# HarrisonKramer/optiland

Hardware: NVIDIA H100
Metric: ray-surface intersections/sec (higher is better)
Workload: dtype f32

## Files before the change

__graft_entry__.py:

```python
from __future__ import annotations

import os
import subprocess
import sys

ROOT = os.path.dirname(os.path.abspath(__file__))
if ROOT not in sys.path:
    sys.path.insert(0, ROOT)

CSRC = os.path.join(ROOT, "optiland_b200", "csrc")
LIB = os.path.join(ROOT, "optiland_b200", "libolb.so")
NVCC_FLAGS = [
    "-gencode", "arch=compute_90a,code=sm_90a", "-lineinfo", "-O3", "-std=c++17",
    "--shared", "-Xcompiler", "-fPIC",
]


def _stale(target: str, deps: list[str]) -> bool:
    if not os.path.exists(target):
        return True
    t = os.path.getmtime(target)
    return any(os.path.getmtime(d) > t for d in deps)


def build(force: bool = False) -> None:
    deps = [os.path.join(CSRC, f) for f in ("olb_trace.cu", "olb_math.cuh", "olb_prep.h", "olb_psf.cu", "olb_fftpsf.cuh",
                                            "olb_irradiance.cu", "olb_irradiance.cuh", "olb_bsdf.cuh", "olb_aim.cuh")]
    deps.append(os.path.join(ROOT, "include", "olb.h"))
    if force or _stale(LIB, deps):
        nvcc = os.environ.get("NVCC", "/usr/local/cuda/bin/nvcc")
        cmd = [nvcc, *NVCC_FLAGS, "-o", LIB, os.path.join(CSRC, "olb_trace.cu"), os.path.join(CSRC, "olb_psf.cu"),
               os.path.join(CSRC, "olb_irradiance.cu")]
        print("[build]", " ".join(cmd), flush=True)
        subprocess.check_call(cmd)
    hc_src = os.path.join(ROOT, "tests", "hostcheck", "hostcheck.cpp")
    hc_so = os.path.join(ROOT, "tests", "hostcheck", "_hostcheck.so")
    if force or _stale(hc_so, [hc_src] + deps[1:3] + [deps[4]]):
        subprocess.check_call(["g++", "-O2", "-std=c++17", "-mfma", "-ffp-contract=fast", "-shared", "-fPIC", "-o", hc_so, hc_src])
    from oracle import hostcheck_phase

    hostcheck_phase.build(force)
    from oracle import hostcheck_grating

    hostcheck_grating.build(force)
    from oracle import hostcheck_coating

    hostcheck_coating.build(force)
    from oracle import hostcheck_grid_sag

    hostcheck_grid_sag.build(force)
    from oracle import hostcheck_polygon

    hostcheck_polygon.build(force)
    from oracle import hostcheck_bsdf

    hostcheck_bsdf.build(force)
    from oracle import hostcheck_aim

    hostcheck_aim.build(force)
    from oracle import hostcheck_irradiance

    hostcheck_irradiance.build(force)
    subprocess.check_call(["bash", os.path.join(ROOT, "oracle", "make_ref.sh")])
    import optiland_b200
    from optiland_b200 import _lib

    _lib.load()


def smoke() -> None:
    import numpy as np
    import torch

    from oracle import trace_oracle as O
    from optiland_b200.trace import RealRays, SurfaceGroup
    from tests._util import REC, Case, max_abs_err

    assert torch.cuda.is_available(), "smoke() needs a CUDA device"
    c = Case("dgauss_c2")
    _, orec, _ = O.trace(c.table, c.rays)
    for dtype, tol in ((torch.float64, 1e-11 * c.scale), (torch.float32, 2e-6 * c.scale)):
        sg = SurfaceGroup(c.table, device="cuda:0")
        r = c.rays
        rays = RealRays(r["x"], r["y"], r["z"], r["L"], r["M"], r["N"], r["i"], r["w"], dtype=dtype, device="cuda:0")
        sg.trace(rays)
        torch.cuda.synchronize()
        for k in REC:
            got = getattr(sg, k).double().cpu().numpy()
            err_o = max_abs_err(got, orec[k])
            err_g = max_abs_err(got, c.rec[k])
            assert err_o <= tol and err_g <= tol, (str(dtype), k, err_o, err_g, tol)
        print(f"[smoke] {dtype}: 13 surfaces x {c.n} rays match oracle + golden within {tol:.2e} mm")
    from oracle.ref_import import reference_available

    if reference_available():
        from oracle.ref_import import import_reference

        import_reference()
        import optiland.backend as be
        from optiland.samples.objectives import DoubleGauss

        from optiland_b200 import _lib, plugin

        be.set_backend("numpy")
        ref = DoubleGauss()
        ref.trace(Hx=0.0, Hy=0.7, wavelength=0.5876, num_rays=8, distribution="hexapolar")
        want = np.array(ref.surfaces.y)
        be.set_backend("torch")
        be.set_device("cuda")
        be.set_precision("float64")
        be.grad_mode.disable()
        plugin.install()
        try:
            l0 = _lib.load().olb_launch_count()
            lens = DoubleGauss()
            lens.trace(Hx=0.0, Hy=0.7, wavelength=0.5876, num_rays=8, distribution="hexapolar")
            got = be.to_numpy(lens.surfaces.y)
            assert _lib.load().olb_launch_count() > l0 and not plugin.stats(), plugin.stats()
            assert np.max(np.abs(got - want)) <= 1e-11 * c.scale
            print("[smoke] unmodified Optic.trace through the plugin == NumPy reference (one fused launch)")
        finally:
            plugin.uninstall()
            be.set_device("cpu")
            be.set_backend("numpy")
    print("[smoke] ok")


if __name__ == "__main__":
    build()
    if len(sys.argv) > 1 and sys.argv[1] == "smoke":
        smoke()
```

include/olb.h:

```cpp
#ifndef OLB_H_
#define OLB_H_

#include <stdint.h>

#ifdef __cplusplus
extern "C" {
#endif

#define OLB_VERSION_MAJOR 0
#define OLB_VERSION_MINOR 3

#define OLB_OK                 0
#define OLB_ERR_INVALID_ARG   -1
#define OLB_ERR_UNSUPPORTED   -2
#define OLB_ERR_CUDA          -3
#define OLB_ERR_ALIGNMENT     -4
#define OLB_ERR_TABLE         -5

#define OLB_GEOM_NOOP          0
#define OLB_GEOM_PLANE         1
#define OLB_GEOM_STANDARD      2
#define OLB_GEOM_EVEN_ASPHERE  3
#define OLB_GEOM_ZERNIKE       4
#define OLB_GEOM_ODD_ASPHERE   5
#define OLB_GEOM_POLYNOMIAL    6
#define OLB_GEOM_CHEBYSHEV     7
#define OLB_GEOM_BICONIC       8
#define OLB_GEOM_TOROIDAL      9
#define OLB_GEOM_FORBES_QBFS  10
#define OLB_GEOM_GRID_SAG     11
#define OLB_MAX_GRID_ELEMENTS 8192


#define OLB_SF_REFLECT     (1u << 0)
#define OLB_SF_ROTATED     (1u << 1)
#define OLB_SF_APERTURE    (1u << 2)
#define OLB_SF_ABSORBING   (1u << 3)
#define OLB_SF_NORECORD    (1u << 4)
#define OLB_SF_BSDF        (1u << 5)

#define OLB_BSDF_LAMBERTIAN 1
#define OLB_BSDF_GAUSSIAN   2
#define OLB_BSDF_MAX_ATTEMPTS 65536

#define OLB_COAT_NONE      0
#define OLB_COAT_SIMPLE    1
#define OLB_COAT_FRESNEL   2
#define OLB_COAT_THIN_FILM 3
#define OLB_COAT_POLARIZER 4
#define OLB_COAT_RETARDER  5
#define OLB_MAX_FILM_LAYERS 32

#define OLB_INTERACT_REFRACT        0
#define OLB_INTERACT_PHASE_CONSTANT 1
#define OLB_INTERACT_PHASE_LINEAR   2
#define OLB_INTERACT_PHASE_RADIAL   3
#define OLB_INTERACT_GRATING        4
#define OLB_MAX_PHASE_TERMS        16

#define OLB_AP_RADIAL      1
#define OLB_AP_OFFSET_RADIAL 2
#define OLB_AP_RECT        3
#define OLB_AP_ELLIPSE     4
#define OLB_AP_POLYGON     5
#define OLB_AP_UNION       16
#define OLB_AP_INTERSECT   17
#define OLB_AP_DIFFERENCE  18
#define OLB_MAX_POLYGON_VERTICES 1024

#define OLB_TF_POLARIZED   (1u << 0)
#define OLB_TF_POL_IDENTITY (1u << 2)
#define OLB_TF_SHARED_INPUT (1u << 4)
#define OLB_TF_MOMENTS     (1u << 3)
#define OLB_TF_MOMENTS_GLOBAL (1u << 5)
#define OLB_TF_MOMENTS_ALL (1u << 6)
#define OLB_TF_NO_FINAL    (1u << 1)

#define OLB_MAX_SURFACES   64
#define OLB_MAX_WAVELENGTHS 16

typedef struct OlbSurface {
  int32_t kind;
  uint32_t flags;
  int32_t n_coef;
  int32_t coef_off;
  int32_t aper_off;
  int32_t aper_len;
  int32_t max_iter;
  int32_t coating;
  int32_t media_off;
  int32_t aux0;
  int32_t interaction;
  int32_t phase_off;
  double t[3];
  double R[9];
  double radius;
  double conic;
  double tol;
  double coat_t;
  double coat_r;
  double norm_radius;
} OlbSurface;


typedef struct OlbTable {
  const OlbSurface* surfaces;
  int32_t n_surfaces;
  int32_t n_wl;
  const double* wavelengths;
  const double* pool;
  int32_t pool_len;
  int32_t reserved;
} OlbTable;

typedef struct OlbRays {
  void* x; void* y; void* z;
  void* L; void* M; void* N;
  void* i; void* w; void* opd;
  void* L0; void* M0; void* N0;
  void* p;
} OlbRays;

typedef struct OlbRecords {
  void* x; void* y; void* z;
  void* L; void* M; void* N;
  void* intensity; void* opd;
  int64_t row_stride;
} OlbRecords;

#define OLB_ST_CHEBYSHEV_RANGE (1 << 1)
#define OLB_ST_ZERNIKE_RANGE (1 << 0)

#define OLB_ST_K_PARALLEL_X (1 << 2)
#define OLB_ST_BSDF_ATTEMPTS (1 << 3)
#define OLB_ST_AIM_NAN_START (1 << 4)
#define OLB_ST_AIM_UNCONVERGED (1 << 5)

int olb_version(void);
int olb_last_error(char* buf, int buf_len);

typedef struct OlbDeviceTable {
  void* workspace;
  int64_t workspace_bytes;
  uint32_t magic;
  uint32_t features;
  int32_t n_surfaces;
  int32_t n_wl;
  int32_t off_f64, bytes_f64;
  int32_t off_f32, bytes_f32;
  int32_t bwd_supported;
  int32_t bwd_slots;
  int32_t n_systems;
  int32_t stride_f64;
  int32_t stride_f32;
  int32_t hints;
} OlbDeviceTable;

int64_t olb_table_workspace_bytes(const OlbTable* table);

int olb_table_upload(const OlbTable* table, void* workspace, int64_t workspace_bytes,
                     void* stream, OlbDeviceTable* out);

typedef struct OlbPupilLaunch {
  const void* Px;
  const void* Py;
  double origin0[3];
  double origin_scale[2];
  double target0[3];
  double target_scale[2];
  double intensity;
  const void* Hx;
  const void* Hy;
  int32_t field_mode;
  int32_t n_vig;
  double field_arg;
  double origin_field[2];
  double target_field[2];
  int32_t vig_power;
  int32_t reserved;
  double vig[16][4];
} OlbPupilLaunch;
#define OLB_MAX_VIG_FIELDS 16

int64_t olb_host_scratch_bytes(int32_t elem_size, int64_t chunk_rays);
int olb_trace_host_f32(const OlbDeviceTable* table, int32_t first, int32_t last,
                       const OlbPupilLaunch* launch, const OlbRays* h_in, const OlbRays* h_out,
                       const OlbRecords* rec, int64_t n_rays, int64_t chunk_rays,
                       void* dev_scratch, int64_t dev_scratch_bytes, uint32_t flags,
                       int32_t* status);
int olb_trace_host_f64(const OlbDeviceTable* table, int32_t first, int32_t last,
                       const OlbPupilLaunch* launch, const OlbRays* h_in, const OlbRays* h_out,
                       const OlbRecords* rec, int64_t n_rays, int64_t chunk_rays,
                       void* dev_scratch, int64_t dev_scratch_bytes, uint32_t flags,
                       int32_t* status);

#define OLB_GP_TX 0
#define OLB_GP_TY 1
#define OLB_GP_TZ 2
#define OLB_GP_CURV 3
#define OLB_GP_CONIC 4
#define OLB_GP_N1 5
#define OLB_GP_N2 6
#define OLB_GP_COEF 7
#define OLB_GP_MAX_COEF 12
#define OLB_GP_R (OLB_GP_COEF + OLB_GP_MAX_COEF)
#define OLB_GP_COUNT (OLB_GP_R + 9)

#define OLB_GT_DIM 12
#define OLB_GT_PER_SURFACE (2 * OLB_GT_DIM * OLB_GT_DIM)
int olb_trace_bwd_f32(const OlbDeviceTable* table, int32_t first, int32_t last,
                      const OlbRays* rays_in, const OlbRecords* rec, const OlbRecords* grad_rec,
                      const OlbRays* grad_rays_in, double* grad_params, double* grad_tables, int64_t n_rays,
                      uint64_t grad_row_mask, void* stream);
int olb_trace_bwd_f64(const OlbDeviceTable* table, int32_t first, int32_t last,
                      const OlbRays* rays_in, const OlbRecords* rec, const OlbRecords* grad_rec,
                      const OlbRays* grad_rays_in, double* grad_params, double* grad_tables, int64_t n_rays,
                      uint64_t grad_row_mask, void* stream);

typedef struct {
  double center[3];
  double radius;
  double n_image;
  double tilt[2];
  double opd_ref;
  double wavelength_um;
} OlbWavefrontRef;
typedef struct {
  void* opd;
  void* pupil_x;
  void* pupil_y;
  void* pupil_z;
  void* intensity;
} OlbWavefrontOut;

typedef struct OlbPolarization {
  int32_t is_polarized;
  int32_t reserved;
  double Ex, Ey;
  double phase_x, phase_y;
  void* intensity;
} OlbPolarization;

#define OLB_BP_TX 0
#define OLB_BP_TY 1
#define OLB_BP_TZ 2
#define OLB_BP_R 3
#define OLB_BP_CURV 12
#define OLB_BP_CONIC 13
#define OLB_BP_N1 14
#define OLB_BP_N2 15
#define OLB_BP_COEF 16
#define OLB_BP_MAX_COEF 12
#define OLB_BP_COUNT (OLB_BP_COEF + OLB_BP_MAX_COEF)
int64_t olb_table_batch_workspace_bytes(const OlbTable* template_table, int32_t n_systems);
int olb_table_upload_batch(const OlbTable* template_table, const double* params, int32_t n_systems,
                           void* workspace, int64_t workspace_bytes, void* stream, OlbDeviceTable* out);

typedef struct OlbTraceCall {
  int32_t first, last;
  int64_t n_rays;
  uint32_t flags;
  uint32_t rng_stream;
  const OlbRays* rays;
  const OlbRecords* rec;
  const OlbPupilLaunch* launch;
  double center[2];
  double* moments;
  int64_t rays_per_system;
  const OlbWavefrontRef* wavefront_ref;
  const OlbWavefrontOut* wavefront_out;
  const OlbPolarization* pol;
  int32_t* status;
} OlbTraceCall;
int olb_trace_call_f32(const OlbDeviceTable* table, const OlbTraceCall* call, void* stream);
int olb_trace_call_f64(const OlbDeviceTable* table, const OlbTraceCall* call, void* stream);

typedef struct OlbAimCall {
  int32_t first, last;
  int64_t n_rays;
  const OlbRays* rays;
  const void* Px;
  const void* Py;
  double r_stop;
  double J_factor;
  double tol;
  int32_t max_iter;
  int32_t infinite;
  int32_t* status;
} OlbAimCall;
int olb_aim_f32(const OlbDeviceTable* table, const OlbAimCall* call, void* stream);
int olb_aim_f64(const OlbDeviceTable* table, const OlbAimCall* call, void* stream);

int olb_huygens_psf_f64(const double* image_x, const double* image_y, const double* image_z, int64_t n_image,
                        const double* pupil_x, const double* pupil_y, const double* pupil_z,
                        const double* pupil_amp_re, const double* pupil_amp_im, const double* pupil_opd,
                        int32_t n_pupil, double wavelength_mm, double Rp, double* psf, double* field,
                        void* stream);

int olb_fft_pupil_f64(const double* opd_waves, const double* intensity, int64_t n_samples, const int32_t* cell_ray,
                      int32_t num_rays, int32_t grid_size, double* pupil, void* stream);
int olb_fft_pupil_f32(const float* opd_waves, const float* intensity, int64_t n_samples, const int32_t* cell_ray,
                      int32_t num_rays, int32_t grid_size, float* pupil, void* stream);
int olb_fft_psf_accumulate_f64(const double* amp, int32_t grid_size, int32_t first, int32_t last, double div, double mul,
                               double* psf, void* stream);
int olb_fft_psf_accumulate_f32(const float* amp, int32_t grid_size, int32_t first, int32_t last, double div, double mul,
                               float* psf, void* stream);

#define OLB_IRR_FRAME_TRANSLATE 0
#define OLB_IRR_FRAME_AFFINE    1
#define OLB_IRR_PATH_AUTO   0
#define OLB_IRR_PATH_SHARED 1
#define OLB_IRR_PATH_GLOBAL 2
typedef struct OlbIrradiance {
  const void* x;
  const void* y;
  const void* z;
  const void* i;
  int64_t n_rays;
  int32_t frame;
  int32_t nx, ny;
  int32_t path;
  double t[3];
  double R[9];
  const double* x_edges;
  const double* y_edges;
  double* edges;
  double* hist;
} OlbIrradiance;
int olb_irradiance_f32(const OlbIrradiance* call, void* stream);
int olb_irradiance_f64(const OlbIrradiance* call, void* stream);

int64_t olb_launch_count(void);

#ifdef __cplusplus
}
#endif
#endif
```

optiland_b200/_lib.py:

```python
from __future__ import annotations

import ctypes as C
import os
from functools import lru_cache

import numpy as np

from . import table as T

_HERE = os.path.dirname(os.path.abspath(__file__))
LIB_PATH = os.path.join(_HERE, "libolb.so")

OK = 0
ERRORS = {-1: "OLB_ERR_INVALID_ARG", -2: "OLB_ERR_UNSUPPORTED", -3: "OLB_ERR_CUDA",
          -4: "OLB_ERR_ALIGNMENT", -5: "OLB_ERR_TABLE"}

TF_POLARIZED = 1 << 0
TF_NO_FINAL = 1 << 1
TF_POL_IDENTITY = 1 << 2
TF_MOMENTS = 1 << 3
TF_SHARED_INPUT = 1 << 4
TF_MOMENTS_GLOBAL = 1 << 5
TF_MOMENTS_ALL = 1 << 6
BP_TX, BP_TY, BP_TZ, BP_R, BP_CURV, BP_CONIC, BP_N1, BP_N2, BP_COEF, BP_MAX_COEF = 0, 1, 2, 3, 12, 13, 14, 15, 16, 12
BP_COUNT = BP_COEF + BP_MAX_COEF
GP_TX, GP_TY, GP_TZ, GP_CURV, GP_CONIC, GP_N1, GP_N2, GP_COEF, GP_MAX_COEF = 0, 1, 2, 3, 4, 5, 6, 7, 12
GP_R = GP_COEF + GP_MAX_COEF
GP_COUNT = GP_R + 9
GT_DIM = 12
GT_PER_SURFACE = 2 * GT_DIM * GT_DIM


class OlbTable(C.Structure):
    _fields_ = [
        ("surfaces", C.c_void_p), ("n_surfaces", C.c_int32), ("n_wl", C.c_int32),
        ("wavelengths", C.c_void_p), ("pool", C.c_void_p), ("pool_len", C.c_int32),
        ("reserved", C.c_int32),
    ]


class OlbRays(C.Structure):
    _fields_ = [(n, C.c_void_p) for n in
                ("x", "y", "z", "L", "M", "N", "i", "w", "opd", "L0", "M0", "N0", "p")]


class OlbRecords(C.Structure):
    _fields_ = [(n, C.c_void_p) for n in ("x", "y", "z", "L", "M", "N", "intensity", "opd")] + [
        ("row_stride", C.c_int64)]


class OlbPupilLaunch(C.Structure):
    _fields_ = [("Px", C.c_void_p), ("Py", C.c_void_p), ("origin0", C.c_double * 3), ("origin_scale", C.c_double * 2),
                ("target0", C.c_double * 3), ("target_scale", C.c_double * 2), ("intensity", C.c_double),
                ("Hx", C.c_void_p), ("Hy", C.c_void_p), ("field_mode", C.c_int32), ("n_vig", C.c_int32),
                ("field_arg", C.c_double), ("origin_field", C.c_double * 2), ("target_field", C.c_double * 2),
                ("vig_power", C.c_int32), ("reserved", C.c_int32), ("vig", (C.c_double * 4) * 16)]


class OlbWavefrontRef(C.Structure):
    _fields_ = [("center", C.c_double * 3), ("radius", C.c_double), ("n_image", C.c_double), ("tilt", C.c_double * 2),
                ("opd_ref", C.c_double), ("wavelength_um", C.c_double)]


class OlbWavefrontOut(C.Structure):
    _fields_ = [(n, C.c_void_p) for n in ("opd", "pupil_x", "pupil_y", "pupil_z", "intensity")]


class OlbPolarization(C.Structure):
    _fields_ = [("is_polarized", C.c_int32), ("reserved", C.c_int32), ("Ex", C.c_double), ("Ey", C.c_double),
                ("phase_x", C.c_double), ("phase_y", C.c_double), ("intensity", C.c_void_p)]


class OlbTraceCall(C.Structure):
    _fields_ = [("first", C.c_int32), ("last", C.c_int32), ("n_rays", C.c_int64), ("flags", C.c_uint32),
                ("rng_stream", C.c_uint32), ("rays", C.POINTER(OlbRays)), ("rec", C.POINTER(OlbRecords)),
                ("launch", C.POINTER(OlbPupilLaunch)), ("center", C.c_double * 2), ("moments", C.c_void_p),
                ("rays_per_system", C.c_int64), ("wavefront_ref", C.POINTER(OlbWavefrontRef)),
                ("wavefront_out", C.POINTER(OlbWavefrontOut)), ("pol", C.POINTER(OlbPolarization)),
                ("status", C.c_void_p)]


class OlbAimCall(C.Structure):
    _fields_ = [("first", C.c_int32), ("last", C.c_int32), ("n_rays", C.c_int64), ("rays", C.POINTER(OlbRays)),
                ("Px", C.c_void_p), ("Py", C.c_void_p), ("r_stop", C.c_double), ("J_factor", C.c_double),
                ("tol", C.c_double), ("max_iter", C.c_int32), ("infinite", C.c_int32), ("status", C.c_void_p)]


class OlbIrradiance(C.Structure):
    _fields_ = [("x", C.c_void_p), ("y", C.c_void_p), ("z", C.c_void_p), ("i", C.c_void_p), ("n_rays", C.c_int64),
                ("frame", C.c_int32), ("nx", C.c_int32), ("ny", C.c_int32), ("path", C.c_int32),
                ("t", C.c_double * 3), ("R", C.c_double * 9), ("x_edges", C.c_void_p), ("y_edges", C.c_void_p),
                ("edges", C.c_void_p), ("hist", C.c_void_p)]


IRR_FRAME_TRANSLATE, IRR_FRAME_AFFINE = 0, 1
IRR_PATH_AUTO, IRR_PATH_SHARED, IRR_PATH_GLOBAL = 0, 1, 2


class OlbDeviceTable(C.Structure):
    _fields_ = [
        ("workspace", C.c_void_p), ("workspace_bytes", C.c_int64), ("magic", C.c_uint32),
        ("features", C.c_uint32), ("n_surfaces", C.c_int32), ("n_wl", C.c_int32),
        ("off_f64", C.c_int32), ("bytes_f64", C.c_int32), ("off_f32", C.c_int32),
        ("bytes_f32", C.c_int32), ("bwd_supported", C.c_int32), ("bwd_slots", C.c_int32),
        ("n_systems", C.c_int32), ("stride_f64", C.c_int32), ("stride_f32", C.c_int32), ("hints", C.c_int32),
    ]


_P = C.POINTER
SYMBOLS = {
    "olb_version": (C.c_int, []),
    "olb_last_error": (C.c_int, [C.c_char_p, C.c_int]),
    "olb_launch_count": (C.c_int64, []),
    "olb_table_workspace_bytes": (C.c_int64, [_P(OlbTable)]),
    "olb_table_upload": (C.c_int, [_P(OlbTable), C.c_void_p, C.c_int64, C.c_void_p, _P(OlbDeviceTable)]),
    "olb_trace_call_f32": (C.c_int, [_P(OlbDeviceTable), _P(OlbTraceCall), C.c_void_p]),
    "olb_trace_call_f64": (C.c_int, [_P(OlbDeviceTable), _P(OlbTraceCall), C.c_void_p]),
    "olb_aim_f32": (C.c_int, [_P(OlbDeviceTable), _P(OlbAimCall), C.c_void_p]),
    "olb_aim_f64": (C.c_int, [_P(OlbDeviceTable), _P(OlbAimCall), C.c_void_p]),
    "olb_trace_bwd_f32": (C.c_int, [_P(OlbDeviceTable), C.c_int32, C.c_int32, _P(OlbRays), _P(OlbRecords),
                                    _P(OlbRecords), _P(OlbRays), C.c_void_p, C.c_void_p, C.c_int64, C.c_uint64,
                                    C.c_void_p]),
    "olb_trace_bwd_f64": (C.c_int, [_P(OlbDeviceTable), C.c_int32, C.c_int32, _P(OlbRays), _P(OlbRecords),
                                    _P(OlbRecords), _P(OlbRays), C.c_void_p, C.c_void_p, C.c_int64, C.c_uint64,
                                    C.c_void_p]),
    "olb_table_batch_workspace_bytes": (C.c_int64, [_P(OlbTable), C.c_int32]),
    "olb_table_upload_batch": (C.c_int, [_P(OlbTable), C.c_void_p, C.c_int32, C.c_void_p, C.c_int64, C.c_void_p,
                                         _P(OlbDeviceTable)]),
    "olb_huygens_psf_f64": (C.c_int, [C.c_void_p, C.c_void_p, C.c_void_p, C.c_int64, C.c_void_p, C.c_void_p, C.c_void_p,
                                      C.c_void_p, C.c_void_p, C.c_void_p, C.c_int32, C.c_double, C.c_double,
                                      C.c_void_p, C.c_void_p, C.c_void_p]),
    "olb_fft_pupil_f64": (C.c_int, [C.c_void_p, C.c_void_p, C.c_int64, C.c_void_p, C.c_int32, C.c_int32, C.c_void_p, C.c_void_p]),
    "olb_fft_pupil_f32": (C.c_int, [C.c_void_p, C.c_void_p, C.c_int64, C.c_void_p, C.c_int32, C.c_int32, C.c_void_p, C.c_void_p]),
    "olb_fft_psf_accumulate_f64": (C.c_int, [C.c_void_p, C.c_int32, C.c_int32, C.c_int32, C.c_double, C.c_double, C.c_void_p, C.c_void_p]),
    "olb_fft_psf_accumulate_f32": (C.c_int, [C.c_void_p, C.c_int32, C.c_int32, C.c_int32, C.c_double, C.c_double, C.c_void_p, C.c_void_p]),
    "olb_irradiance_f32": (C.c_int, [_P(OlbIrradiance), C.c_void_p]),
    "olb_irradiance_f64": (C.c_int, [_P(OlbIrradiance), C.c_void_p]),
    "olb_host_scratch_bytes": (C.c_int64, [C.c_int32, C.c_int64]),
    "olb_trace_host_f32": (C.c_int, [_P(OlbDeviceTable), C.c_int32, C.c_int32, _P(OlbPupilLaunch), _P(OlbRays),
                                     _P(OlbRays), _P(OlbRecords), C.c_int64, C.c_int64, C.c_void_p, C.c_int64,
                                     C.c_uint32, C.c_void_p]),
    "olb_trace_host_f64": (C.c_int, [_P(OlbDeviceTable), C.c_int32, C.c_int32, _P(OlbPupilLaunch), _P(OlbRays),
                                     _P(OlbRays), _P(OlbRecords), C.c_int64, C.c_int64, C.c_void_p, C.c_int64,
                                     C.c_uint32, C.c_void_p]),
}


class OlbError(RuntimeError):
    pass


@lru_cache(maxsize=1)
def load() -> C.CDLL:
    if not os.path.exists(LIB_PATH):
        raise OlbError(
            f"{LIB_PATH} not found: build it with `python -c 'import __graft_entry__ as g; g.build()'` "
            "(nvcc, sm_90a).  optiland_b200 has no CPU fallback.")
    lib = C.CDLL(LIB_PATH)
    for name, (restype, argtypes) in SYMBOLS.items():
        fn = getattr(lib, name)
        fn.restype = restype
        fn.argtypes = argtypes
    return lib


def last_error() -> str:
    buf = C.create_string_buffer(512)
    load().olb_last_error(buf, len(buf))
    return buf.value.decode("utf-8", "replace")


def check(rc: int, what: str) -> None:
    if rc != OK:
        raise OlbError(f"{what} failed: {ERRORS.get(rc, rc)}: {last_error()}")


class HostTable:

    def __init__(self, tab: T.SurfaceTable, packed=None):
        self.surf, self.pool = packed if packed is not None else tab.pack()
        self.surf = np.ascontiguousarray(self.surf)
        self.pool = np.ascontiguousarray(self.pool)
        self.wl = np.ascontiguousarray(tab.wavelengths, dtype=np.float64)
        self.c = OlbTable(
            surfaces=self.surf.ctypes.data, n_surfaces=len(self.surf), n_wl=len(self.wl),
            wavelengths=self.wl.ctypes.data, pool=self.pool.ctypes.data, pool_len=len(self.pool),
            reserved=0)
```

optiland_b200/trace.py:

```python
from __future__ import annotations

import ctypes as C
import threading

import numpy as np
import torch

from . import _lib
from . import table as T

_REC_KEYS = ("x", "y", "z", "L", "M", "N", "intensity", "opd")
_DTYPES = {torch.float32: "f32", torch.float64: "f64"}
_CDTYPES = {torch.float32: torch.complex64, torch.float64: torch.complex128}


def _require_cuda():
    if not torch.cuda.is_available():
        raise _lib.OlbError("optiland_b200 needs a CUDA device (sm_90a); there is no CPU fallback")


def _as_dev(v, n, dtype, device):
    t = torch.as_tensor(v, dtype=dtype, device=device)
    if t.ndim == 0:
        t = t.expand(n)
    t = t.reshape(-1).contiguous()
    if t.data_ptr() % 16:
        t = t.clone()
    return t


class RealRays:

    def __init__(self, x, y, z, L, M, N, intensity, wavelength, dtype=torch.float32, device=None):
        _require_cuda()
        if dtype not in _DTYPES:
            raise ValueError("dtype must be torch.float32 or torch.float64")
        device = torch.device(device if device is not None else f"cuda:{torch.cuda.current_device()}")
        n = max(int(np.size(v)) if not torch.is_tensor(v) else v.numel()
                for v in (x, y, z, L, M, N, intensity, wavelength))
        self.x = _as_dev(x, n, dtype, device)
        self.y = _as_dev(y, n, dtype, device)
        self.z = _as_dev(z, n, dtype, device)
        self.L = _as_dev(L, n, dtype, device)
        self.M = _as_dev(M, n, dtype, device)
        self.N = _as_dev(N, n, dtype, device)
        self.i = _as_dev(intensity, n, dtype, device)
        self.w = _as_dev(wavelength, n, dtype, device)
        self.opd = torch.zeros_like(self.x)
        self.L0 = self.M0 = self.N0 = None
        self.is_normalized = True

    def __len__(self):
        return self.x.numel()

    @property
    def dtype(self):
        return self.x.dtype

    @property
    def device(self):
        return self.x.device


class PolarizedRays(RealRays):

    def __init__(self, x, y, z, L, M, N, intensity, wavelength, dtype=torch.float32, device=None):
        super().__init__(x, y, z, L, M, N, intensity, wavelength, dtype=dtype, device=device)
        self.p = None
        self._i0 = self.i.clone()
        self._L0, self._M0, self._N0 = self.L.clone(), self.M.clone(), self.N.clone()

    def update_intensity(self, state=None):
        k = torch.stack([self._L0, self._M0, self._N0], dim=1)
        xh = torch.tensor([1.0, 0.0, 0.0], dtype=k.dtype, device=k.device).expand_as(k)
        pv = torch.linalg.cross(k, xh)
        norms = torch.linalg.norm(pv, dim=1)
        if bool((norms == 0).any()):
            raise ValueError("k-vector parallel to x-axis is not currently supported.")
        pv = pv / norms[:, None]
        sv = torch.linalg.cross(pv, k)
        states = [state] if state is not None else [(1.0, 0.0, 0.0, 0.0), (0.0, 1.0, 0.0, 0.0)]
        inten = torch.zeros_like(self._i0)
        P = self.p
        for Ex, Ey, phx, phy in states:
            ax = complex(np.cos(phx), np.sin(phx)) * Ex
            ay = complex(np.cos(phy), np.sin(phy)) * Ey
            E0 = sv.to(P.dtype) * ax + pv.to(P.dtype) * ay
            E1 = torch.matmul(P, E0[:, :, None])[:, :, 0]
            inten = inten + (E1.abs() ** 2).sum(dim=1)
        self.i = inten * self._i0 / len(states)


class DeviceTable:

    DEFAULT_WORKSPACE = 48 * 1024

    def __init__(self, table: T.SurfaceTable, device=None, packed=None):
        _require_cuda()
        self.lib = _lib.load()
        self.table = table
        self.device = torch.device(device if device is not None else f"cuda:{torch.cuda.current_device()}")
        self.host = _lib.HostTable(table, packed)
        self.c = _lib.OlbDeviceTable()
        nbytes = self.DEFAULT_WORKSPACE
        for attempt in range(2):
            self.workspace = torch.empty(int(nbytes), dtype=torch.uint8, device=self.device)
            with torch.cuda.device(self.device):
                stream = torch.cuda.current_stream(self.device).cuda_stream
                rc = self.lib.olb_table_upload(C.byref(self.host.c), self.workspace.data_ptr(), int(nbytes),
                                               C.c_void_p(stream), C.byref(self.c))
            if rc != 0 and attempt == 0 and "workspace too small" in _lib.last_error():
                nbytes = self.lib.olb_table_workspace_bytes(C.byref(self.host.c))
                if nbytes < 0:
                    _lib.check(int(nbytes), "olb_table_workspace_bytes")
                continue
            break
        _lib.check(rc, "olb_table_upload")
        self.ready = torch.cuda.Event()
        self.ready.record(torch.cuda.current_stream(self.device))
        self.has_zernike = any(s.kind in (T.GEOM_ZERNIKE, T.GEOM_CHEBYSHEV) for s in table.surfaces)
        self.has_bsdf = any(s.bsdf != T.BSDF_NONE for s in table.surfaces)

    @property
    def features(self) -> int:
        return int(self.c.features)


def _byref(s):
    return C.byref(s) if s is not None else None


def _pointer(s):
    return C.pointer(s) if s is not None else None


def _status_word(dtab: "DeviceTable", device, force: bool = False):
    return torch.zeros(1, dtype=torch.int32, device=device) if (dtab.has_zernike or _has_bsdf(dtab) or force) else None


def _has_bsdf(dtab) -> bool:
    return getattr(dtab, "has_bsdf", False)


_STREAM = {"state": None, "next": 0}
_STREAM_LOCK = threading.Lock()


def next_rng_stream() -> int:
    g = torch.default_generator
    with _STREAM_LOCK:
        st = g.get_state()
        if _STREAM["state"] is None or not torch.equal(st, _STREAM["state"]):
            _STREAM["next"] = int(torch.randint(0, 1 << 32, (1,), dtype=torch.int64).item())
            _STREAM["state"] = g.get_state()
        s = _STREAM["next"]
        _STREAM["next"] = (s + 1) & 0xFFFFFFFF
        return s


def _raise_status(status) -> None:
    if status is None:
        return
    st = int(status.item())
    if st & T.ST_ZERNIKE_RANGE:
        raise ValueError(
            "Zernike coordinates must be normalized to [-1, 1]. Consider updating the normalization "
            "radius to 1.1x the surface aperture.")
    if st & T.ST_CHEBYSHEV_RANGE:
        raise ValueError(
            "Chebyshev input coordinates must be normalized to [-1, 1]. Consider updating the "
            "normalization factors.")
    if st & T.ST_K_PARALLEL_X:
        raise ValueError("k-vector parallel to x-axis is not currently supported.")
    if st & T.ST_BSDF_ATTEMPTS:
        raise ValueError(f"BSDF scatter: a ray rejected {T.BSDF_MAX_ATTEMPTS} drawn directions (is the Gaussian sigma "
                         "far above 1?); its direction is NaN")


def _out_buffer(k: int, rows: int, n: int, dtype, device) -> torch.Tensor:
    vec = 4 if dtype == torch.float32 else 2
    stride = n if n % vec == 0 else (n + 63) // 64 * 64
    return torch.empty((k, rows, stride), dtype=dtype, device=device)


def _c_records(buf: torch.Tensor):
    return _lib.OlbRecords(*[buf[j].data_ptr() for j in range(8)], buf.shape[-1])


def _take_last_row(rays, recs):
    rays.x, rays.y, rays.z = recs["x"][-1], recs["y"][-1], recs["z"][-1]
    rays.L, rays.M, rays.N = recs["L"][-1], recs["M"][-1], recs["N"][-1]
    rays.i, rays.opd = recs["intensity"][-1], recs["opd"][-1]
    return rays


def _trace(dtab, device, dtype, first, last, n, flags, rays=None, rec=None, launch=None, center=(0.0, 0.0),
           moments=None, rays_per_system=0, wavefront=None, pol=None, status=None, own_status=True, rng_stream=None):
    if _has_bsdf(dtab) and rng_stream is None:
        rng_stream = next_rng_stream()
    if own_status:
        status = _status_word(dtab, device, force=pol is not None)
    ref, out = wavefront if wavefront is not None else (None, None)
    call = _lib.OlbTraceCall(
        first=first, last=last, n_rays=n, flags=flags, rng_stream=int(rng_stream or 0), rays=_pointer(rays),
        rec=_pointer(rec), launch=_pointer(launch),
        center=(float(center[0]), float(center[1])), moments=moments.data_ptr() if moments is not None else None,
        rays_per_system=rays_per_system, wavefront_ref=_pointer(ref), wavefront_out=_pointer(out), pol=_pointer(pol),
        status=status.data_ptr() if status is not None else None)
    sfx = _DTYPES[dtype]
    with torch.cuda.device(device):
        stream = torch.cuda.current_stream(device).cuda_stream
        rc = getattr(dtab.lib, f"olb_trace_call_{sfx}")(C.byref(dtab.c), C.byref(call), C.c_void_p(stream))
    _lib.check(rc, f"olb_trace_call_{sfx}")
    if own_status:
        _raise_status(status)


def _c_polarization(state, intensity_out=None):
    c = _lib.OlbPolarization()
    if state is None or state == "unpolarized":
        c.is_polarized = 0
    else:
        Ex, Ey, phx, phy = (float(v) for v in state)
        mag = (Ex * Ex + Ey * Ey) ** 0.5
        c.is_polarized, c.Ex, c.Ey, c.phase_x, c.phase_y = 1, Ex / mag, Ey / mag, phx, phy
    c.intensity = intensity_out.data_ptr() if intensity_out is not None else None
    return c


def trace_device(dtab: DeviceTable, rays: RealRays, first: int, last: int, record: bool = True,
                 want_l0: bool = False, polarization=False, rng_stream=None):
    n = len(rays)
    if rays.device != dtab.device:
        raise ValueError(f"rays on {rays.device}, table on {dtab.device}")
    rows = last - first
    recs = None
    c_rec = None
    flags = 0
    if record and rows > 0:
        buf = _out_buffer(8, rows, n, rays.dtype, rays.device)
        recs = {k: buf[j, :, :n] for j, k in enumerate(_REC_KEYS)}
        c_rec = _c_records(buf)
        flags |= _lib.TF_NO_FINAL
    if want_l0:
        rays.L0 = torch.empty_like(rays.x)
        rays.M0 = torch.empty_like(rays.x)
        rays.N0 = torch.empty_like(rays.x)
    p_ptr = None
    if isinstance(rays, PolarizedRays):
        flags |= _lib.TF_POLARIZED
        if rays.p is None:
            rays.p = torch.empty((n, 3, 3), dtype=_CDTYPES[rays.dtype], device=rays.device)
            flags |= _lib.TF_POL_IDENTITY
        else:
            rays.p = rays.p.to(_CDTYPES[rays.dtype]).contiguous()
        p_ptr = torch.view_as_real(rays.p).data_ptr()
    c_rays = _lib.OlbRays(
        x=rays.x.data_ptr(), y=rays.y.data_ptr(), z=rays.z.data_ptr(), L=rays.L.data_ptr(),
        M=rays.M.data_ptr(), N=rays.N.data_ptr(), i=rays.i.data_ptr(),
        w=rays.w.data_ptr() if dtab.table.n_wl > 1 else None, opd=rays.opd.data_ptr(),
        L0=rays.L0.data_ptr() if want_l0 else None, M0=rays.M0.data_ptr() if want_l0 else None,
        N0=rays.N0.data_ptr() if want_l0 else None, p=p_ptr)
    pol_i, c_pol = None, None
    if polarization is not False:
        if not isinstance(rays, PolarizedRays):
            raise ValueError("the intensity epilogue needs PolarizedRays")
        pol_i = torch.empty_like(rays.x)
        c_pol = _c_polarization(polarization, pol_i)
    _trace(dtab, rays.device, rays.dtype, first, last, n, flags, rays=c_rays, rec=c_rec, pol=c_pol, rng_stream=rng_stream)
    if recs is not None:
        _take_last_row(rays, recs)
    if pol_i is not None:
        rays.i = pol_i
    return recs


def aim_device(dtab: DeviceTable, guess: dict, Px: torch.Tensor, Py: torch.Tensor, first: int, last: int,
               r_stop: float, J_factor: float, tol: float, max_iter: int, infinite: bool) -> torch.Tensor:
    x = guess["x"]
    n = int(x.numel())
    for t in [guess[k] for k in ("y", "z", "L", "M", "N")] + [Px, Py]:
        if t.dtype != x.dtype or t.device != dtab.device or t.numel() != n:
            raise ValueError("aim: guess and pupil arrays must share one dtype, length and the table's device")
    status = torch.zeros(1, dtype=torch.int32, device=dtab.device)
    w = guess.get("w") if dtab.table.n_wl > 1 else None
    c_rays = _lib.OlbRays(x=x.data_ptr(), y=guess["y"].data_ptr(), z=guess["z"].data_ptr(), L=guess["L"].data_ptr(),
                          M=guess["M"].data_ptr(), N=guess["N"].data_ptr(), w=w.data_ptr() if w is not None else None)
    call = _lib.OlbAimCall(first=first, last=last, n_rays=n, rays=C.pointer(c_rays), Px=Px.data_ptr(), Py=Py.data_ptr(),
                           r_stop=float(r_stop), J_factor=float(J_factor), tol=float(tol), max_iter=int(max_iter),
                           infinite=1 if infinite else 0, status=status.data_ptr())
    sfx = _DTYPES[x.dtype]
    with torch.cuda.device(dtab.device):
        stream = torch.cuda.current_stream(dtab.device).cuda_stream
        rc = getattr(dtab.lib, f"olb_aim_{sfx}")(C.byref(dtab.c), C.byref(call), C.c_void_p(stream))
    _lib.check(rc, f"olb_aim_{sfx}")
    return status


def _aligned(t):
    if t is None:
        return None
    t = t.contiguous()
    return t.clone() if t.data_ptr() % 16 else t


def _c_launch(affine: dict, Px, Py):
    la = _lib.OlbPupilLaunch()
    la.Px, la.Py = Px.data_ptr(), Py.data_ptr()
    la.origin0 = (C.c_double * 3)(*affine["origin0"])
    la.origin_scale = (C.c_double * 2)(*affine["origin_scale"])
    la.target0 = (C.c_double * 3)(*affine["target0"])
    la.target_scale = (C.c_double * 2)(*affine["target_scale"])
    la.intensity = float(affine.get("intensity", 1.0))
    fields = affine.get("fields")
    if fields is not None:
        Hx, Hy = fields
        la.Hx, la.Hy = Hx.data_ptr(), Hy.data_ptr()
        la.field_mode = int(affine["field_mode"])
        la.field_arg = float(affine.get("field_arg", 0.0))
        la.origin_field = (C.c_double * 2)(*affine["origin_field"])
        la.target_field = (C.c_double * 2)(*affine["target_field"])
        vig = affine.get("vig")
        if vig is not None:
            tab, power = vig
            tab = np.asarray(tab, dtype=np.float64).reshape(-1, 4)
            if len(tab) > 16:
                raise ValueError("more than 16 defined fields with vignetting factors")
            la.n_vig, la.vig_power = len(tab), int(power)
            for j, row in enumerate(tab):
                for q in range(4):
                    la.vig[j][q] = float(row[q])
    return la


def trace_pupil_device(dtab: DeviceTable, Px: torch.Tensor, Py: torch.Tensor, affine: dict, first: int, last: int,
                       wavelength: torch.Tensor | None = None, polarization=False):
    Px, Py, wavelength = _aligned(Px), _aligned(Py), _aligned(wavelength)
    if affine.get("fields") is not None:
        affine = dict(affine, fields=tuple(_aligned(t) for t in affine["fields"]))
    n, dtype, dev = Px.numel(), Px.dtype, Px.device
    buf = _out_buffer(8, last - first, n, dtype, dev)
    recs = {k: buf[j, :, :n] for j, k in enumerate(_REC_KEYS)}
    la = _c_launch(affine, Px.contiguous(), Py.contiguous())
    out = _lib.OlbRays(w=wavelength.data_ptr() if (wavelength is not None and dtab.table.n_wl > 1) else None)
    flags = _lib.TF_NO_FINAL
    p, inten, c_pol = None, None, None
    if polarization is not False:
        flags |= _lib.TF_POLARIZED
        p = torch.empty((n, 3, 3), dtype=_CDTYPES[dtype], device=dev)
        out.p = torch.view_as_real(p).data_ptr()
        if polarization != "matrix":
            inten = torch.empty(n, dtype=dtype, device=dev)
            c_pol = _c_polarization(polarization, inten)
    _trace(dtab, dev, dtype, first, last, n, flags, rays=out, rec=_c_records(buf), launch=la, pol=c_pol)
    cls = RealRays if p is None else PolarizedRays
    rays = _take_last_row(cls.__new__(cls), recs)
    if p is not None:
        rays.p = p
    if inten is not None:
        rays.i = inten
    rays.w = wavelength
    rays.L0 = rays.M0 = rays.N0 = None
    rays.is_normalized = True
    return rays, recs


WAVEFRONT_KEYS = ("opd", "pupil_x", "pupil_y", "pupil_z", "intensity")


def trace_wavefront_device(dtab: DeviceTable, Px: torch.Tensor, Py: torch.Tensor, affine: dict, ref: dict,
                           wavelength: torch.Tensor | None = None, polarized: bool = False) -> dict:
    Px, Py, wavelength = _aligned(Px), _aligned(Py), _aligned(wavelength)
    n, dtype, dev = Px.numel(), Px.dtype, Px.device
    buf = _out_buffer(5, 1, n, dtype, dev)[:, 0]
    c_out = _lib.OlbWavefrontOut(*[buf[j].data_ptr() for j in range(5)])
    c_ref = _lib.OlbWavefrontRef()
    c_ref.center = (C.c_double * 3)(*[float(v) for v in ref["center"]])
    c_ref.radius, c_ref.n_image = float(ref["radius"]), float(ref["n_image"])
    c_ref.tilt = (C.c_double * 2)(*[float(v) for v in ref.get("tilt", (0.0, 0.0))])
    c_ref.opd_ref, c_ref.wavelength_um = float(ref["opd_ref"]), float(ref["wavelength_um"])
    la = _c_launch(affine, Px.contiguous(), Py.contiguous())
    rays = _lib.OlbRays(w=wavelength.data_ptr() if (wavelength is not None and dtab.table.n_wl > 1) else None)
    flags = _lib.TF_NO_FINAL
    p = None
    if polarized:
        flags |= _lib.TF_POLARIZED
        p = torch.empty((n, 3, 3), dtype=_CDTYPES[dtype], device=dev)
        rays.p = torch.view_as_real(p).data_ptr()
    _trace(dtab, dev, dtype, 0, dtab.table.num_surfaces, n, flags, rays=rays, launch=la, wavefront=(c_ref, c_out))
    out = {k: buf[j, :n] for j, k in enumerate(WAVEFRONT_KEYS)}
    if p is not None:
        out["p"] = p
    return out


def trace_moments_device(dtab: DeviceTable, n: int, dtype, rays: RealRays | None = None, pupil=None,
                         center=(0.0, 0.0), moments: torch.Tensor | None = None, wavelength=None,
                         status: torch.Tensor | None = None, last: int | None = None, global_xy: bool = False,
                         every_ray: bool = False) -> torch.Tensor:
    dev = dtab.device
    if moments is None:
        moments = torch.zeros(8, dtype=torch.float64, device=dev)
    la = None
    c_rays = _lib.OlbRays()
    if pupil is not None:
        Px, Py, affine = pupil
        Px, Py, wavelength = _aligned(Px), _aligned(Py), _aligned(wavelength)
        la = _c_launch(affine, Px, Py)
        if wavelength is not None and dtab.table.n_wl > 1:
            c_rays.w = wavelength.data_ptr()
    else:
        for k in ("x", "y", "z", "L", "M", "N", "i", "opd"):
            setattr(c_rays, k, getattr(rays, k).data_ptr())
        if dtab.table.n_wl > 1:
            c_rays.w = rays.w.data_ptr()
    flags = _lib.TF_NO_FINAL | (_lib.TF_MOMENTS_GLOBAL if global_xy else 0) | (_lib.TF_MOMENTS_ALL if every_ray else 0)
    _trace(dtab, dev, dtype, 0, dtab.table.num_surfaces if last is None else last, n, flags, rays=c_rays, launch=la,
           center=center, moments=moments, status=status, own_status=status is None)
    return moments


def moments_to_spot(m, center=(0.0, 0.0)) -> dict:
    m = [float(v) for v in (m.cpu() if torch.is_tensor(m) else m)]
    cnt = m[0]
    if cnt == 0:
        return {"count": 0.0}
    mx, my = m[1] / cnt, m[2] / cnt
    var_c = max(m[3] / cnt - mx * mx - my * my, 0.0)
    opd_mean = m[5] / cnt
    return {"count": cnt, "centroid": (center[0] + mx, center[1] + my), "rms_centroid": var_c ** 0.5,
            "rms_center": (m[3] / cnt) ** 0.5, "intensity_sum": m[4], "opd_mean": opd_mean,
            "opd_rms": max(m[6] / cnt - opd_mean * opd_mean, 0.0) ** 0.5}


class SurfaceGroup:

    def __init__(self, table: T.SurfaceTable, device=None):
        self.table = table
        self.device_table = DeviceTable(table, device)
        self._rec = None

    @property
    def num_surfaces(self) -> int:
        return self.table.num_surfaces

    def trace(self, rays: RealRays, skip: int = 0, stop: int | None = None, record: bool = True):
        last = self.num_surfaces if stop is None else stop
        if not 0 <= skip <= last <= self.num_surfaces:
            raise ValueError("bad surface range")
        self._rec = trace_device(self.device_table, rays, skip, last, record=record)
        return rays

    def trace_pupil(self, Px, Py, affine: dict, wavelength=None):
        rays, self._rec = trace_pupil_device(self.device_table, Px, Py, affine, 0, self.num_surfaces, wavelength)
        return rays

    def spot_moments(self, rays=None, pupil=None, center=(0.0, 0.0), dtype=None):
        if pupil is not None:
            n, dt = pupil[0].numel(), pupil[0].dtype
        else:
            n, dt = len(rays), rays.dtype
        m = trace_moments_device(self.device_table, n, dtype or dt, rays=rays, pupil=pupil, center=center)
        out = moments_to_spot(m, center)
        cen = out.get("centroid")
        if cen is not None and np.isfinite(cen[0]) and np.isfinite(cen[1]):
            m2 = trace_moments_device(self.device_table, n, dtype or dt, rays=rays, pupil=pupil, center=cen)
            out["rms_centroid"] = moments_to_spot(m2, cen)["rms_centroid"]
        return out

    def _get(self, key):
        if self._rec is None:
            raise RuntimeError("no records: call trace(..., record=True) first")
        return self._rec[key]

    x = property(lambda self: self._get("x"))
    y = property(lambda self: self._get("y"))
    z = property(lambda self: self._get("z"))
    L = property(lambda self: self._get("L"))
    M = property(lambda self: self._get("M"))
    N = property(lambda self: self._get("N"))
    opd = property(lambda self: self._get("opd"))
    intensity = property(lambda self: self._get("intensity"))


def trace_host(dtab: DeviceTable, h_in: dict, h_out: dict, n: int, dtype=torch.float32, chunk: int = 1 << 20,
               scratch: torch.Tensor | None = None, rec=None, first: int = 0, last: int | None = None,
               affine: dict | None = None):
    lib = dtab.lib
    sfx = _DTYPES[dtype]
    es = 4 if dtype == torch.float32 else 8
    last = dtab.table.num_surfaces if last is None else last
    dtab.ready.synchronize()
    need = int(lib.olb_host_scratch_bytes(es, chunk))
    if scratch is None or scratch.numel() < need:
        scratch = torch.empty(need, dtype=torch.uint8, device=dtab.device)
    c_out = _lib.OlbRays(**{k: h_out[k].data_ptr() for k in ("x", "y", "z", "L", "M", "N", "i", "opd")})
    la, c_in = None, None
    if affine is not None:
        la = _c_launch(affine, h_in["Px"], h_in["Py"])
        if dtab.table.n_wl > 1:
            c_out.w = (h_in["w"] if "w" in h_in else h_out["w"]).data_ptr()
    else:
        c_in = _lib.OlbRays(**{k: h_in[k].data_ptr() for k in ("x", "y", "z", "L", "M", "N", "i")},
                            w=h_in["w"].data_ptr() if "w" in h_in and dtab.table.n_wl > 1 else None)
    c_rec = _c_records(rec) if rec is not None else None
    status = torch.zeros(1, dtype=torch.int32, device=dtab.device) if _has_bsdf(dtab) else None
    with torch.cuda.device(dtab.device):
        rc = getattr(lib, f"olb_trace_host_{sfx}")(
            C.byref(dtab.c), first, last, _byref(la), _byref(c_in), C.byref(c_out), _byref(c_rec), n, chunk,
            C.c_void_p(scratch.data_ptr()), scratch.numel(), 0,
            C.c_void_p(status.data_ptr()) if status is not None else None)
    _lib.check(rc, f"olb_trace_host_{sfx}")
    _raise_status(status)
    return scratch
```

Baseline: 72.94 billion.

## Allocate uniform ray arrays in compressible device memory via pluggable allocator

Adds a CUDA driver-API allocator that requests generic-compression memory through cuMemCreate and exposes it to PyTorch as a MemPool. When RealRays builds its input arrays, any freshly created array whose values are all equal (for example wavelength, intensity or the zeroed OPD) is copied into this compressible memory. The aim is to cut DRAM bandwidth for these reads using hardware compression of uniform data. In exchange it adds a uniformity check with a host sync at construction, a full-device synchronize on every free, and VMM allocation overhead.

```diff
diff --git a/__graft_entry__.py b/__graft_entry__.py
--- a/__graft_entry__.py
+++ b/__graft_entry__.py
@@ -25,12 +25,13 @@
 
 def build(force: bool = False) -> None:
     deps = [os.path.join(CSRC, f) for f in ("olb_trace.cu", "olb_math.cuh", "olb_prep.h", "olb_psf.cu", "olb_fftpsf.cuh",
-                                            "olb_irradiance.cu", "olb_irradiance.cuh", "olb_bsdf.cuh", "olb_aim.cuh")]
+                                            "olb_irradiance.cu", "olb_irradiance.cuh", "olb_bsdf.cuh", "olb_aim.cuh",
+                                            "olb_alloc.cu")]
     deps.append(os.path.join(ROOT, "include", "olb.h"))
     if force or _stale(LIB, deps):
         nvcc = os.environ.get("NVCC", "/usr/local/cuda/bin/nvcc")
         cmd = [nvcc, *NVCC_FLAGS, "-o", LIB, os.path.join(CSRC, "olb_trace.cu"), os.path.join(CSRC, "olb_psf.cu"),
-               os.path.join(CSRC, "olb_irradiance.cu")]
+               os.path.join(CSRC, "olb_irradiance.cu"), os.path.join(CSRC, "olb_alloc.cu")]
         print("[build]", " ".join(cmd), flush=True)
         subprocess.check_call(cmd)
     hc_src = os.path.join(ROOT, "tests", "hostcheck", "hostcheck.cpp")
diff --git a/include/olb.h b/include/olb.h
--- a/include/olb.h
+++ b/include/olb.h
@@ -1,6 +1,7 @@
 #ifndef OLB_H_
 #define OLB_H_
 
+#include <stddef.h>
 #include <stdint.h>
 
 #ifdef __cplusplus
@@ -332,6 +333,11 @@
 
 int64_t olb_launch_count(void);
 
+int olb_compressible_supported(int device);
+void* olb_compressible_alloc(size_t size, int device, void* stream);
+void olb_compressible_free(void* ptr, size_t size, int device, void* stream);
+int olb_compressible_stats(int device, int64_t* granted_bytes, int64_t* plain_bytes);
+
 #ifdef __cplusplus
 }
 #endif
diff --git a/optiland_b200/_lib.py b/optiland_b200/_lib.py
--- a/optiland_b200/_lib.py
+++ b/optiland_b200/_lib.py
@@ -143,6 +143,10 @@
     "olb_trace_host_f64": (C.c_int, [_P(OlbDeviceTable), C.c_int32, C.c_int32, _P(OlbPupilLaunch), _P(OlbRays),
                                      _P(OlbRays), _P(OlbRecords), C.c_int64, C.c_int64, C.c_void_p, C.c_int64,
                                      C.c_uint32, C.c_void_p]),
+    "olb_compressible_supported": (C.c_int, [C.c_int]),
+    "olb_compressible_alloc": (C.c_void_p, [C.c_size_t, C.c_int, C.c_void_p]),
+    "olb_compressible_free": (None, [C.c_void_p, C.c_size_t, C.c_int, C.c_void_p]),
+    "olb_compressible_stats": (C.c_int, [C.c_int, _P(C.c_int64), _P(C.c_int64)]),
 }
 
 
diff --git a/optiland_b200/csrc/olb_alloc.cu b/optiland_b200/csrc/olb_alloc.cu
--- /dev/null
+++ b/optiland_b200/csrc/olb_alloc.cu
@@ -0,0 +1,179 @@
+#include <cuda.h>
+#include <cuda_runtime.h>
+#include <stdint.h>
+
+#include <mutex>
+#include <unordered_map>
+
+#include "../../include/olb.h"
+
+namespace olb {
+int fail_psf(int code, const char* msg);
+
+namespace {
+
+struct Driver {
+  decltype(&cuDeviceGet) DeviceGet = nullptr;
+  decltype(&cuDeviceGetAttribute) DeviceGetAttribute = nullptr;
+  decltype(&cuMemGetAllocationGranularity) MemGetAllocationGranularity = nullptr;
+  decltype(&cuMemCreate) MemCreate = nullptr;
+  decltype(&cuMemGetAllocationPropertiesFromHandle) MemGetAllocationPropertiesFromHandle = nullptr;
+  decltype(&cuMemAddressReserve) MemAddressReserve = nullptr;
+  decltype(&cuMemMap) MemMap = nullptr;
+  decltype(&cuMemSetAccess) MemSetAccess = nullptr;
+  decltype(&cuMemUnmap) MemUnmap = nullptr;
+  decltype(&cuMemRelease) MemRelease = nullptr;
+  decltype(&cuMemAddressFree) MemAddressFree = nullptr;
+  bool ok = false;
+};
+
+template <class F>
+bool entry(const char* name, F& fn) {
+  cudaDriverEntryPointQueryResult q;
+  void* p = nullptr;
+  if (cudaGetDriverEntryPointByVersion(name, &p, 12000, cudaEnableDefault, &q) != cudaSuccess ||
+      q != cudaDriverEntryPointSuccess || p == nullptr)
+    return false;
+  fn = reinterpret_cast<F>(p);
+  return true;
+}
+
+const Driver& driver() {
+  static Driver d;
+  static std::once_flag once;
+  std::call_once(once, [] {
+    int n = 0;
+    if (cudaGetDeviceCount(&n) != cudaSuccess || n == 0) return;
+    d.ok = entry("cuDeviceGet", d.DeviceGet) && entry("cuDeviceGetAttribute", d.DeviceGetAttribute) &&
+           entry("cuMemGetAllocationGranularity", d.MemGetAllocationGranularity) &&
+           entry("cuMemCreate", d.MemCreate) &&
+           entry("cuMemGetAllocationPropertiesFromHandle", d.MemGetAllocationPropertiesFromHandle) &&
+           entry("cuMemAddressReserve", d.MemAddressReserve) && entry("cuMemMap", d.MemMap) &&
+           entry("cuMemSetAccess", d.MemSetAccess) && entry("cuMemUnmap", d.MemUnmap) &&
+           entry("cuMemRelease", d.MemRelease) && entry("cuMemAddressFree", d.MemAddressFree);
+  });
+  return d;
+}
+
+struct Mapping {
+  CUmemGenericAllocationHandle handle;
+  size_t bytes;
+  int device;
+  bool compressed;
+};
+
+struct Stats {
+  int64_t granted = 0;
+  int64_t plain = 0;
+};
+
+std::mutex g_mu;
+std::unordered_map<uintptr_t, Mapping> g_maps;
+std::unordered_map<int, Stats> g_stats;
+
+}
+}
+
+using namespace olb;
+
+extern "C" {
+
+int olb_compressible_supported(int device) {
+  const Driver& d = driver();
+  CUdevice dev;
+  int v = 0;
+  if (!d.ok || d.DeviceGet(&dev, device) != CUDA_SUCCESS ||
+      d.DeviceGetAttribute(&v, CU_DEVICE_ATTRIBUTE_GENERIC_COMPRESSION_SUPPORTED, dev) != CUDA_SUCCESS)
+    return 0;
+  return v != 0;
+}
+
+void* olb_compressible_alloc(size_t size, int device, void* stream) {
+  (void)stream;
+  const Driver& d = driver();
+  if (!d.ok) {
+    fail_psf(OLB_ERR_CUDA, "olb_compressible_alloc: driver entry points unavailable");
+    return nullptr;
+  }
+  CUmemAllocationProp prop = {};
+  prop.type = CU_MEM_ALLOCATION_TYPE_PINNED;
+  prop.location.type = CU_MEM_LOCATION_TYPE_DEVICE;
+  prop.location.id = device;
+  prop.allocFlags.compressionType = CU_MEM_ALLOCATION_COMP_GENERIC;
+  size_t gran = 0;
+  if (d.MemGetAllocationGranularity(&gran, &prop, CU_MEM_ALLOC_GRANULARITY_RECOMMENDED) != CUDA_SUCCESS || gran == 0) {
+    fail_psf(OLB_ERR_CUDA, "olb_compressible_alloc: cuMemGetAllocationGranularity failed");
+    return nullptr;
+  }
+  const size_t bytes = (size + gran - 1) / gran * gran;
+  CUmemGenericAllocationHandle h;
+  if (d.MemCreate(&h, bytes, &prop, 0) != CUDA_SUCCESS) {
+    fail_psf(OLB_ERR_CUDA, "olb_compressible_alloc: cuMemCreate failed");
+    return nullptr;
+  }
+  CUdeviceptr ptr = 0;
+  if (d.MemAddressReserve(&ptr, bytes, gran, 0, 0) != CUDA_SUCCESS) {
+    d.MemRelease(h);
+    fail_psf(OLB_ERR_CUDA, "olb_compressible_alloc: cuMemAddressReserve failed");
+    return nullptr;
+  }
+  if (d.MemMap(ptr, bytes, 0, h, 0) != CUDA_SUCCESS) {
+    d.MemAddressFree(ptr, bytes);
+    d.MemRelease(h);
+    fail_psf(OLB_ERR_CUDA, "olb_compressible_alloc: cuMemMap failed");
+    return nullptr;
+  }
+  CUmemAccessDesc access = {};
+  access.location = prop.location;
+  access.flags = CU_MEM_ACCESS_FLAGS_PROT_READWRITE;
+  if (d.MemSetAccess(ptr, bytes, &access, 1) != CUDA_SUCCESS) {
+    d.MemUnmap(ptr, bytes);
+    d.MemAddressFree(ptr, bytes);
+    d.MemRelease(h);
+    fail_psf(OLB_ERR_CUDA, "olb_compressible_alloc: cuMemSetAccess failed");
+    return nullptr;
+  }
+  CUmemAllocationProp got = {};
+  const bool compressed = d.MemGetAllocationPropertiesFromHandle(&got, h) == CUDA_SUCCESS &&
+                          got.allocFlags.compressionType == CU_MEM_ALLOCATION_COMP_GENERIC;
+  std::lock_guard<std::mutex> lk(g_mu);
+  g_maps[(uintptr_t)ptr] = Mapping{h, bytes, device, compressed};
+  Stats& s = g_stats[device];
+  (compressed ? s.granted : s.plain) += (int64_t)bytes;
+  return (void*)ptr;
+}
+
+void olb_compressible_free(void* ptr, size_t size, int device, void* stream) {
+  (void)size;
+  (void)stream;
+  Mapping m;
+  {
+    std::lock_guard<std::mutex> lk(g_mu);
+    auto it = g_maps.find((uintptr_t)ptr);
+    if (it == g_maps.end()) return;
+    m = it->second;
+    g_maps.erase(it);
+    Stats& s = g_stats[m.device];
+    (m.compressed ? s.granted : s.plain) -= (int64_t)m.bytes;
+  }
+  int prev = 0;
+  cudaGetDevice(&prev);
+  cudaSetDevice(device);
+  cudaDeviceSynchronize();
+  cudaSetDevice(prev);
+  const Driver& d = driver();
+  d.MemUnmap((CUdeviceptr)ptr, m.bytes);
+  d.MemAddressFree((CUdeviceptr)ptr, m.bytes);
+  d.MemRelease(m.handle);
+}
+
+int olb_compressible_stats(int device, int64_t* granted_bytes, int64_t* plain_bytes) {
+  if (!granted_bytes || !plain_bytes) return fail_psf(OLB_ERR_INVALID_ARG, "granted_bytes or plain_bytes is NULL");
+  std::lock_guard<std::mutex> lk(g_mu);
+  auto it = g_stats.find(device);
+  *granted_bytes = it == g_stats.end() ? 0 : it->second.granted;
+  *plain_bytes = it == g_stats.end() ? 0 : it->second.plain;
+  return OLB_OK;
+}
+
+}
diff --git a/optiland_b200/trace.py b/optiland_b200/trace.py
--- a/optiland_b200/trace.py
+++ b/optiland_b200/trace.py
@@ -1,6 +1,8 @@
 from __future__ import annotations
 
+import contextlib
 import ctypes as C
+import os
 import threading
 
 import numpy as np
@@ -17,6 +19,56 @@
 def _require_cuda():
     if not torch.cuda.is_available():
         raise _lib.OlbError("optiland_b200 needs a CUDA device (sm_90a); there is no CPU fallback")
+
+
+_POOLS: dict = {}
+_POOLS_LOCK = threading.Lock()
+
+
+def _compressible_pool(index: int):
+    with _POOLS_LOCK:
+        if index not in _POOLS:
+            pool = None
+            if _lib.load().olb_compressible_supported(index):
+                alloc = torch.cuda.memory.CUDAPluggableAllocator(_lib.LIB_PATH, "olb_compressible_alloc",
+                                                                 "olb_compressible_free")
+                with torch.cuda.device(index):
+                    pool = torch.cuda.MemPool(alloc.allocator())
+            _POOLS[index] = pool
+        return _POOLS[index]
+
+
+def _pool_of(device: torch.device):
+    if device.type != "cuda" or os.environ.get("OLB_COMPRESSIBLE", "1") == "0" or not torch.cuda.is_available():
+        return None
+    index = device.index if device.index is not None else torch.cuda.current_device()
+    pool = _compressible_pool(index)
+    return (pool, index) if pool is not None else None
+
+
+@contextlib.contextmanager
+def compressible(device):
+    pool = _pool_of(torch.device(device))
+    if pool is None:
+        yield
+        return
+    with torch.cuda.use_mem_pool(*pool):
+        yield
+
+
+def _uniform_to_compressible(arrays: list, fresh: list, device: torch.device) -> list:
+    if _pool_of(device) is None:
+        return arrays
+    cand = [j for j, t in enumerate(arrays) if fresh[j]]
+    if not cand:
+        return arrays
+    uniform = torch.stack([(arrays[j] == arrays[j][:1]).all() for j in cand]).tolist()
+    out = list(arrays)
+    with compressible(device):
+        for j, u in zip(cand, uniform):
+            if u:
+                out[j] = torch.empty_like(arrays[j]).copy_(arrays[j])
+    return out
 
 
 def _as_dev(v, n, dtype, device):
@@ -38,15 +90,11 @@
         device = torch.device(device if device is not None else f"cuda:{torch.cuda.current_device()}")
         n = max(int(np.size(v)) if not torch.is_tensor(v) else v.numel()
                 for v in (x, y, z, L, M, N, intensity, wavelength))
-        self.x = _as_dev(x, n, dtype, device)
-        self.y = _as_dev(y, n, dtype, device)
-        self.z = _as_dev(z, n, dtype, device)
-        self.L = _as_dev(L, n, dtype, device)
-        self.M = _as_dev(M, n, dtype, device)
-        self.N = _as_dev(N, n, dtype, device)
-        self.i = _as_dev(intensity, n, dtype, device)
-        self.w = _as_dev(wavelength, n, dtype, device)
-        self.opd = torch.zeros_like(self.x)
+        src = (x, y, z, L, M, N, intensity, wavelength)
+        arrays = [_as_dev(v, n, dtype, device) for v in src] + [torch.zeros(n, dtype=dtype, device=device)]
+        fresh = [not (torch.is_tensor(v) and v.data_ptr() == t.data_ptr()) for v, t in zip(src, arrays)] + [True]
+        (self.x, self.y, self.z, self.L, self.M, self.N, self.i, self.w,
+         self.opd) = _uniform_to_compressible(arrays, fresh, device)
         self.L0 = self.M0 = self.N0 = None
         self.is_normalized = True
 
```

Result: faster. 74.50 billion (median of 6 runs) (+2.1%).
